# aharley/pips

Hardware: AMD Instinct MI355X
Metric: particle-updates/sec (B*S*N*iters/s) at S=8 N=256 368x496 (higher is better)
Workload: dtype f32; 1 GPU; BASELINE configs[1]: B=1/GPU S=8 368x496 N=256 I=6 fp32 stride 8, encoder included, inputs resident in HBM; clips_per_gpu=1, parallelism=clip-sharded x1, collective=none

## Files before the change

__graft_entry__.py:

```python
from __future__ import annotations

import os
import sys

ROOT = os.path.dirname(os.path.abspath(__file__))
if ROOT not in sys.path:
    sys.path.insert(0, ROOT)


def build() -> None:
    from pips_amd import _build
    lib = _build.build_library()
    assert os.path.exists(lib)
    import pips_amd
    from pips_amd import _lib
    _lib.load()
    from oracle import reference_shim
    if reference_shim.available() and os.environ.get("PIPS_SKIP_REF_CHECK") != "1":
        import subprocess
        subprocess.check_call([sys.executable, os.path.join(ROOT, "oracle", "check_against_reference.py")])


def smoke() -> None:
    import torch
    from pips_amd import Pips
    from pips_amd.weights import init_state_dict
    from oracle import pips_oracle as O

    assert torch.cuda.is_available(), "smoke() needs cuda:0"
    sd = init_state_dict(0, tamed=True)
    g = torch.Generator().manual_seed(1)
    B, N, H, W, iters = 1, 16, 128, 160, 3
    rgbs = torch.randint(0, 256, (B, 8, 3, H, W), generator=g).float()
    xys = torch.rand(B, N, 2, generator=g) * torch.tensor([W - 1.0, H - 1.0])
    m = Pips(S=8, stride=8)
    m.load_state_dict(sd)
# ... 15 lines not shown
```

pips_amd/csrc/api.hip:

```cpp
#include "common.h"

#include <cstdarg>
#include <cstdio>
#include <cstdlib>
#include <cstring>
#include <mutex>

namespace pips {

static thread_local char g_err[512] = "";

void set_error(const char* fmt, ...) {
    va_list ap;
    va_start(ap, fmt);
    vsnprintf(g_err, sizeof(g_err), fmt, ap);
    va_end(ap);
}

#ifdef PIPS_TUNING
int tune_env(const char* name, int dflt) {
    const char* e = getenv(name);
    return e ? atoi(e) : dflt;
}
#endif
// ... 367 lines not shown
}
const float* conv_w(const float* arena, const ArenaLayout& A, int ci, MatMode mode) {
    if (mode == EXACT) return arena + A.conv[ci].w;
    const unsigned short* hb = reinterpret_cast<const unsigned short*>(arena + A.total);
    return reinterpret_cast<const float*>(mode == BF16 ? hb + A.h_conv[ci] : hb + A.total_h + A.t_conv[ci]);
}

struct Enc {
    const float* arena; const ArenaLayout& A;
    int F; float* ws; const EncPlan& P; hipStream_t st; MatMode mode;
};

ConvCall enc_conv(const Enc& e, int ci, const void* in, int H, int W, void* out, bool out_bf16) {
    const ConvW& c = e.A.conv[ci];
    const MatMode lm = layer_mm(c, e.F, H, W, e.mode);
    ConvCall cc = conv_call(in, e.F, H, W, c.cin, conv_w(e.arena, e.A, ci, lm), e.arena + c.b, c.cout, c.k, c.stride, c.pad, out,
                            nullptr, nullptr);
    cc.mode = lm;
    cc.in_bf16 = e.mode == BF16;
    cc.out_bf16 = out_bf16;
    return cc;
}

int conv_stats(const Enc& e, int ci, const void* in, const float* in_norm, int H, int W, void* out, float* partial,
               float* mean_rstd) {
    const ConvW& c = e.A.conv[ci];
    int tiles = 0;
    ConvCall cc = enc_conv(e, ci, in, H, W, out, e.mode == BF16);
    cc.stats = partial; cc.tiles = &tiles; cc.in_norm = in_norm;
    if (e.mode == BF16) cc.parts_cap = enc_parts_cap(conv_out(H, c.k, c.stride, c.pad), conv_out(W, c.k, c.stride, c.pad));
    RUN(conv_nhwc(cc, e.st));
    return launch_inorm_finalize_pivot(partial, e.F, tiles, c.cout, mean_rstd, e.st);
}

int inorm_apply(const Enc& e, const void* x, const float* stats, const void* res, const float* res_stats, void* y, int HW, int C) {
    if (e.mode == BF16)
        return launch_inorm_apply_bf16(x, stats, res, res_stats, res == nullptr ? 0 : res_stats == nullptr ? 1 : 2, y, e.F, HW, C, e.st);
    return launch_inorm_apply((const float*)x, stats, (const float*)res, res_stats, (float*)y, e.F, HW, C, e.st);
}

int res_block(const Enc& e, int& ci, bool down, const void* x, int H, int W, void* out) {
    const int i1 = ci++, i2 = ci++;
    const ConvW& c1 = e.A.conv[i1];
    const ConvW& c2 = e.A.conv[i2];
    const int Ho = conv_out(H, 3, c1.stride, 1), Wo = conv_out(W, 3, c1.stride, 1);
    float* ws = e.ws; const EncPlan& P = e.P;
    void* raw = ws + P.raw; void* mid = ws + P.mid;
    RUN(conv_stats(e, i1, x, nullptr, H, W, raw, ws + P.partial, ws + P.st_a));
    RUN(inorm_apply(e, raw, ws + P.st_a, nullptr, nullptr, mid, Ho * Wo, c1.cout));
    RUN(conv_stats(e, i2, mid, nullptr, Ho, Wo, raw, ws + P.partial, ws + P.st_a));
    if (down) {
        const int id = ci++;
        RUN(conv_stats(e, id, x, nullptr, H, W, ws + P.ds, ws + P.partial2, ws + P.st_b));
        return inorm_apply(e, raw, ws + P.st_a, ws + P.ds, ws + P.st_b, out, Ho * Wo, c2.cout);
    }
    return inorm_apply(e, raw, ws + P.st_a, x, nullptr, out, Ho * Wo, c2.cout);
}

int enc_front_f32(const Enc& e, const void* rgbs, int rgb_u8, int H, int W, int& ci) {
    float* ws = e.ws; const EncPlan& P = e.P;
    const int H0 = P.Hs[0], W0 = P.Ws[0];
    int tiles = 0;
    RUN(launch_stem(rgbs, rgb_u8, e.arena + e.A.conv[0].w, e.arena + e.A.conv[0].b, ws + P.raw, ws + P.partial, e.F, H, W, H0, W0,
                    &tiles, e.st));
    RUN(launch_inorm_finalize_pivot(ws + P.partial, e.F, tiles, 64, ws + P.st_a, e.st));
    RUN(launch_inorm_apply(ws + P.raw, ws + P.st_a, nullptr, nullptr, ws + P.xa, e.F, H0 * W0, 64, e.st));
    RUN(res_block(e, ci, false, ws + P.xa, H0, W0, ws + P.xb));
    return res_block(e, ci, false, ws + P.xb, H0, W0, ws + P.outs[0]);
}

int enc_front_bf16(const Enc& e, const void* rgbs, int rgb_u8, int H, int W, int& ci) {
    float* ws = e.ws; const EncPlan& P = e.P; const ArenaLayout& A = e.A; hipStream_t st = e.st;
// ... 22 lines not shown
    RUN(check_geometry(F, H, W, stride));
    const EncPlan P = plan_encoder(F, H, W, stride);
    if (workspace_bytes < P.total * sizeof(float)) {
        set_error("encoder: workspace %zu < %zu bytes", workspace_bytes, P.total * sizeof(float));
        return PIPS_E_WORKSPACE;
    }
    float* ws = (float*)workspace;
    const Enc e = {(const float*)arena_v, arena_layout(), F, ws, P, st, encoder_mode(flags)};
    const bool h = e.mode == BF16;
    const int rgb_u8 = (flags & PIPS_FLAG_RGB_U8) ? 1 : 0;

    int ci = 1;
    RUN(h ? enc_front_bf16(e, rgbs, rgb_u8, H, W, ci) : enc_front_f32(e, rgbs, rgb_u8, H, W, ci));
    const void* x = ws + P.outs[0];
    int Hc = P.Hs[0], Wc = P.Ws[0];
    for (int l = 1; l < 4; ++l) {
        RUN(res_block(e, ci, true, x, Hc, Wc, ws + P.xb));
        Hc = P.Hs[l]; Wc = P.Ws[l];
        RUN(res_block(e, ci, false, ws + P.xb, Hc, Wc, ws + P.outs[l]));
        x = ws + P.outs[l];
    }
    const int ch[4] = {64, 96, 128, 128};
    const int H8 = P.Hs[4], W8 = P.Ws[4];
    for (int l = 0, coff = 0; l < 4; coff += ch[l], ++l)
        RUN(h ? launch_resize_into_bf16(ws + P.outs[l], F, P.Hs[l], P.Ws[l], ch[l], ws + P.cat, H8, W8, 416, coff, st)
              : launch_resize_into(ws + P.outs[l], F, P.Hs[l], P.Ws[l], ch[l], ws + P.cat, H8, W8, 416, coff, st));
    const int i2 = ci++, i3 = ci++;
    RUN(conv_stats(e, i2, ws + P.cat, nullptr, H8, W8, ws + P.raw, ws + P.partial, ws + P.st_a));
    RUN(inorm_apply(e, ws + P.raw, ws + P.st_a, nullptr, nullptr, ws + P.mid, H8 * W8, 256));
    RUN(conv_nhwc(enc_conv(e, i3, ws + P.mid, H8, W8, pyramid, false), st));
    const PyramidView v = pyramid_view(F, H8, W8);
    for (int l = 1; l < PIPS_LEVELS; ++l)
        RUN(launch_avgpool2(pyramid + v.off[l - 1], F, v.lh[l - 1], v.lw[l - 1], PIPS_C, pyramid + v.off[l], st));
    if (h) RUN(launch_pyramid_mirror(pyramid, v.levels, pyramid + v.levels, st));
    return PIPS_OK;
}

enum GatherRoute { GATHER_AUTO, GATHER_DIRECT, GATHER_TILED };

struct GatherCall {
    const float* pyramid; int B, T, R, S, H8, W8;
    const float* ffeats; const float* coords; const float* times; int N;
    const int* win_start; const int* win_dir;
    float* X;
    bool bf16_maps; GatherRoute route;
    void* scratch; size_t scratch_bytes; hipEvent_t* ev;
    hipStream_t st;
};

int mixer_input(const GatherCall& g) {
    PIPS_CHECK_ARG(g.pyramid && g.ffeats && g.coords && g.times && g.X, "mixer_input: null pointer");
    PIPS_CHECK_ARG(g.T >= 1 && g.R >= 1 && g.B > 0 && g.N > 0, "mixer_input: need T, R, B, N >= 1");
    PIPS_CHECK_ARG(g.S >= 1 && g.S <= PIPS_S_MAX, "mixer_input: window length S=%d outside 1..%d", g.S, PIPS_S_MAX);
    const PyramidView v = pyramid_view(g.B * g.R, g.H8, g.W8);
// ... 216 lines not shown
    hipStream_t st;
};

int track_impl(const TrackCall& c) {
    PIPS_CHECK_ARG(c.arena && c.pyramid && c.xys && c.times && c.workspace && c.out_trajs && c.out_vis, "track: null pointer");
    PIPS_CHECK_ARG(c.B > 0 && c.N > 0 && c.T >= 1 && c.R >= 1 && c.iters >= 0 && c.stride >= 1,
                   "track: need B,N,T,R,stride >= 1 and iters >= 0");
    PIPS_CHECK_ARG(c.S >= 1 && c.S <= PIPS_S_MAX, "track: window length S=%d outside 1..%d", c.S, PIPS_S_MAX);
    PIPS_CHECK_ARG(c.H8 >= 8 && c.W8 >= 8, "track: map %dx%d too small for a 4-level pyramid", c.H8, c.W8);
    PIPS_CHECK_ARG(c.win_dir == nullptr || c.win_start != nullptr, "track: win_dir needs win_start");
    const int B = c.B, N = c.N, S = c.S;
    const TrackPlan P = plan_track(B, N, S);
    if (c.workspace_bytes < P.total * sizeof(float)) {
        set_error("track: workspace %zu < %zu bytes", c.workspace_bytes, P.total * sizeof(float));
        return PIPS_E_WORKSPACE;
    }
    hipStream_t st = c.st;
    const float* arena = (const float*)c.arena;
    float* ws = (float*)c.workspace;
    const int M = B * N * S;
    float* coords = ws + P.coords; float* coords0 = ws + P.coords0; float* ffeats = ws + P.ffeats;
    float* ffeat0 = c.out_ffeat0 != nullptr ? c.out_ffeat0 : ws + P.ffeat0;
    const size_t traj_sz = (size_t)B * S * N * 2;
    RUN(launch_init_coords(c.xys, c.coords_init, B, N, (float)c.stride, coords, coords0, c.out_trajs, st, S));
    if (c.feat_init != nullptr) {
        if (c.feat_init != ffeat0)
            (void)hipMemcpyAsync(ffeat0, c.feat_init, (size_t)B * N * PIPS_C * sizeof(float), hipMemcpyDeviceToDevice, st);
    } else {
        RUN(launch_point_sample_strided(c.pyramid, B, c.R, c.T, c.H8, c.W8, coords, S * 2, N, c.win_start, ffeat0, st));
    }
    RUN(launch_init_ffeats(ffeat0, B * N, ffeats, st, S));
    if (c.ce_tgt != nullptr) {
        PIPS_CHECK_ARG(c.ce_terms && c.ce_ws && c.win_start == nullptr && c.T == S && c.R == c.T,
                       "track: score-map terms need their output and workspace, S frames per clip and no windows");
        if (c.ce_ws_bytes < score_map_workspace_bytes(B, c.T, c.H8, c.W8)) {
            set_error("track: score-map workspace %zu < %zu bytes", c.ce_ws_bytes, score_map_workspace_bytes(B, c.T, c.H8, c.W8));
            return PIPS_E_WORKSPACE;
        }
        RUN(score_map_prepare(c.pyramid, B, c.T, c.H8, c.W8, (float*)c.ce_ws, st));
    }
    if (c.iters == 0)
        RUN(launch_vis_head(arena, ffeats, B, N, c.out_vis, st, S));
    GatherCall g;
    memset(&g, 0, sizeof(g));
    g.pyramid = c.pyramid; g.B = B; g.T = c.T; g.R = c.R; g.S = S; g.H8 = c.H8; g.W8 = c.W8;
    g.ffeats = ffeats; g.coords = coords; g.times = c.times; g.N = N;
    g.win_start = c.win_start; g.win_dir = c.win_dir;
    g.X = ws + P.X;
    g.bf16_maps = (c.flags & PIPS_FLAG_BF16_MAPS) != 0;
    g.route = GATHER_AUTO;
    g.scratch = ws + P.mixer; g.scratch_bytes = mixer_workspace_bytes(M, S);
    g.st = st;
    for (int it = 0; it < c.iters; ++it) {
        if (c.ce_tgt != nullptr)
// ... 384 lines not shown
```

pips_amd/csrc/common.h:

```cpp
#pragma once
#include <hip/hip_runtime.h>
#include <atomic>
#include <stdint.h>
#include <stddef.h>
#include "../../include/pips_hip.h"

namespace pips {

void set_error(const char* fmt, ...);

#define PIPS_CHECK_ARG(cond, ...)                                   \
    do {                                                            \
        if (!(cond)) { ::pips::set_error(__VA_ARGS__); return PIPS_E_ARG; } \
    } while (0)

#define PIPS_CHECK_LAUNCH(what)                                                     \
    do {                                                                            \
        hipError_t e__ = hipGetLastError();                                         \
        if (e__ != hipSuccess) {                                                    \
            ::pips::set_error("%s: %s", what, hipGetErrorString(e__));              \
            return PIPS_E_LAUNCH;                                                   \
        }                                                                           \
    } while (0)

// ... 237 lines not shown
    size_t w_in, b_in;
    MixLayerW mix[PIPS_DEPTH];
    size_t lnf_g, lnf_b, w_head, b_head;
    size_t norm_g, norm_b, w_upd_t, b_upd, w_vis, b_vis;
    size_t total;
    size_t h_w1[PIPS_DEPTH], h_w2[PIPS_DEPTH], h_head, h_conv[22], h_in, total_h;
    size_t t_in, t_w1[PIPS_DEPTH], t_w2[PIPS_DEPTH], t_head, t_conv[22], total_t;
    int S, nout, nout_pad;
    size_t total_all;
};
const ArenaLayout& arena_layout(int S = PIPS_S);

inline int conv_out(int x, int k, int s, int p) { return (x + 2 * p - k) / s + 1; }

int launch_stem(const void* rgbs, int rgb_u8, const float* w, const float* bias, float* out, float* stats,
                int F, int H, int W, int Ho, int Wo, int* tiles_m, hipStream_t st);
int stem_tiles_m(int Ho, int Wo);
int launch_inorm_finalize_pivot(const float* partial, int F, int parts, int C, float* mean_rstd, hipStream_t st);
int launch_inorm_apply(const float* x, const float* stats, const float* res, const float* res_stats,
                       float* y, int F, int HW, int C, hipStream_t st);
int launch_resize_into(const float* src, int F, int Hs, int Ws, int C, float* dst, int Hd, int Wd,
                       int Cdst, int coff, hipStream_t st);
int launch_avgpool2(const float* src, int F, int H, int W, int C, float* dst, hipStream_t st);
int launch_resize_frames(const void* src, int src_u8, int planes, int h, int w, float* dst, int H, int W, hipStream_t st);
int launch_stem_bf16(const void* rgbs, int rgb_u8, const float* w, const float* bias, void* out_bf16, float* stats,
                     int F, int H, int W, int Ho, int Wo, int* tiles_m, hipStream_t st);
int launch_inorm_apply_bf16(const void* x, const float* stats, const void* res, const float* res_stats, int mode,
                            void* y, int F, int HW, int C, hipStream_t st);
int launch_resize_into_bf16(const void* src, int F, int Hs, int Ws, int C, void* dst, int Hd, int Wd, int Cdst, int coff,
                            hipStream_t st);

int launch_point_sample(const float* level0, int B, int S, int H8, int W8, const float* xy, int N,
                        float* out, hipStream_t st);
int launch_point_sample_strided(const float* level0, int B, int S, int T, int H8, int W8, const float* xy,
                                int xy_stride, int N, const int* win_start, float* out, hipStream_t st);
int launch_init_coords(const float* xys, const float* coords_init, int B, int N, float stride,
                       float* coords, float* coords0, float* out_traj0, hipStream_t st, int Sw = PIPS_S);
int launch_init_ffeats(const float* ffeat0, int BN, float* ffeats, hipStream_t st, int Sw = PIPS_S);
int launch_mixer_input(const float* pyramid, const size_t* lvl_off, const int* lvlH, const int* lvlW,
                       int B, int S, int T, const float* ffeats, const float* coords, const float* times,
                       int N, const int* win_start, const int* win_dir, float* X, hipStream_t st, int Sw = PIPS_S);
int launch_mixer_input_bf16maps(const void* mirror, const size_t* lvl_off, const int* lvlH, const int* lvlW, int B, int S,
                                int T, const float* ffeats, const float* coords, const float* times, int N,
                                const int* win_start, const int* win_dir, float* X, hipStream_t st, int Sw = PIPS_S);
int launch_pyramid_mirror(const float* pyramid, size_t floats, void* mirror, hipStream_t st);
int launch_pyramid_append(const float* src, const size_t* src_off, int k, float* dst, const size_t* dst_off, void* dst_mirror,
                          const int* pf8, int R, int T0, hipStream_t st);
size_t tiled_gather_scratch_bytes(int B, int N, int H8, int W8);
bool tiled_gather_wanted(int B, int N, int H8, int W8, bool bf16_maps = false);
int launch_mixer_input_tiled(const float* pyramid, const size_t* lvl_off, const int* lvlH, const int* lvlW, int B,
                             int S, const float* ffeats, const float* coords, const float* times, int N,
                             float* X, void* scratch, size_t scratch_bytes, hipStream_t st, hipEvent_t* ev = nullptr,
                             const unsigned short* mirror = nullptr);
int launch_token_mix(const float* arena, const MixLayerW& L, float* x, float* xn, int particles,
                     hipStream_t st, int xn_bf16 = 0, int Sw = PIPS_S, int x_bf16 = 0);
int launch_ln_mean(const float* x, const float* g, const float* b, float* out, int particles,
                   hipStream_t st, int Sw = PIPS_S, int x_bf16 = 0);
int launch_score_upsum(const float* pyramid, const size_t* lvl_off, const int* lvlH, const int* lvlW, int F, float* U,
                       hipStream_t st);
int launch_score_terms(const float* U, int B, int S, int H8, int W8, const float* ffeats, int N, const float* tgt,
                       float* out, hipStream_t st);
// ... 7 lines not shown
```

pips_amd/csrc/encoder.hip:

```cpp
#include "common.h"

namespace pips {

constexpr int STEM_ROWS = 4, STEM_COLS = 64;
constexpr int STEM_TH = 2 * STEM_ROWS + 5, STEM_TW = 136;
constexpr int STEM_STEPS = 3 * 7 * 4;
constexpr int STEM_LDS = (3 * STEM_TH * STEM_TW + STEM_STEPS * 64 * 2) * 4;

template <typename RGB, bool V4>
__global__ __launch_bounds__(256, 2) void stem_conv_kernel(const RGB* __restrict__ rgbs,
                                                           const float* __restrict__ w,
                                                           const float* __restrict__ bias,
                                                           float* __restrict__ out,
                                                           float* __restrict__ stats, int H, int W,
                                                           int Ho, int Wo, int tiles_x, int tiles, int F) {
    extern __shared__ __attribute__((aligned(16))) float stem_sm[];
    float* tile = stem_sm;
    float* wl = stem_sm + 3 * STEM_TH * STEM_TW;
    const int tid = threadIdx.x, lane = tid & 63, wave = tid >> 6;
    const int l31 = lane & 31, half = lane >> 5;
    for (int i = tid; i < STEM_STEPS * 64 * 2; i += 256) {
        const int h = i & 1, n = (i >> 1) & 63, s = i >> 7;
        const int j = s & 3, ck = s >> 2, kw = 2 * j + h - (V4 ? 1 : 0);
        wl[i] = (kw >= 0 && kw < 7) ? w[(ck * 7 + kw) * 64 + n] : 0.f;
// ... 109 lines not shown
int launch_stem(const void* rgbs, int rgb_u8, const float* w, const float* bias, float* out, float* stats,
                int F, int H, int W, int Ho, int Wo, int* tiles_m, hipStream_t st) {
    const int tiles_x = cdiv(Wo, STEM_COLS), tiles = cdiv(Ho, STEM_ROWS) * tiles_x;
    if (tiles_m) *tiles_m = stem_tiles_m(Ho, Wo);
    const int grid = tiles * F < 512 ? tiles * F : 512;
    static std::atomic<unsigned long long> raised_f{0}, raised_u{0};
    static std::atomic<unsigned long long> raised_f4{0}, raised_u4{0};
    const bool v4 = W % 4 == 0 && reinterpret_cast<uintptr_t>(rgbs) % (rgb_u8 ? 4 : 16) == 0 && PIPS_TUNE("PIPS_STEM_V4", 1);
#define PIPS_STEM32(T_, V_, RAISED_)                                                                                             \
    {                                                                                                                            \
        const int rc = ensure_dynamic_lds(RAISED_, (const void*)stem_conv_kernel<T_, V_>, STEM_LDS);                            \
        if (rc != PIPS_OK) return rc;                                                                                            \
        hipLaunchKernelGGL((stem_conv_kernel<T_, V_>), dim3(grid), dim3(256), STEM_LDS, st, (const T_*)rgbs, w, bias, out, stats, \
                           H, W, Ho, Wo, tiles_x, tiles, F);                                                                     \
    }
    if (rgb_u8) { if (v4) PIPS_STEM32(unsigned char, true, raised_u4) else PIPS_STEM32(unsigned char, false, raised_u) }
    else { if (v4) PIPS_STEM32(float, true, raised_f4) else PIPS_STEM32(float, false, raised_f) }
#undef PIPS_STEM32
    PIPS_CHECK_LAUNCH("stem_conv_kernel");
    return PIPS_OK;
}

template <int SUBS>
__global__ __launch_bounds__(4 * SUBS) void inorm_finalize_pivot_kernel(const float4* __restrict__ partial, int parts, int C,
                                                                        float* __restrict__ mean_rstd) {
    constexpr int NW = 4 * SUBS / 64;
    __shared__ double red[3][NW][4];
    const int f = blockIdx.x, cl = threadIdx.x & 3, c = blockIdx.y * 4 + cl, sub = threadIdx.x >> 2;
    const float4* p = partial + (size_t)f * parts * C + c;
    const double r = (double)p[0].z;
    double n = 0.0, s1 = 0.0, s2 = 0.0;
    for (int t0 = sub; t0 < parts; t0 += 8 * SUBS) {
        float4 v[8];
#pragma unroll
        for (int u = 0; u < 8; ++u) {
            const int t = t0 + SUBS * u;
            v[u] = t < parts ? p[(size_t)t * C] : make_float4(0.f, 0.f, 0.f, 0.f);
        }
#pragma unroll
        for (int u = 0; u < 8; ++u)
            if (v[u].w > 0.f) {
                const double nt = v[u].w, d = (double)v[u].z - r;
                n += nt;
                s1 += (double)v[u].x + nt * d;
                s2 += (double)v[u].y + d * (2.0 * (double)v[u].x + nt * d);
            }
    }
#pragma unroll
    for (int o = 4; o < 64; o <<= 1) {
        n += __shfl_xor(n, o); s1 += __shfl_xor(s1, o); s2 += __shfl_xor(s2, o);
    }
    const int wave = threadIdx.x >> 6;
    if ((threadIdx.x & 63) < 4) { red[0][wave][cl] = n; red[1][wave][cl] = s1; red[2][wave][cl] = s2; }
    __syncthreads();
    if (threadIdx.x < 4) {
        n = 0.0; s1 = 0.0; s2 = 0.0;
        for (int i = 0; i < NW; ++i) { n += red[0][i][cl]; s1 += red[1][i][cl]; s2 += red[2][i][cl]; }
        const double m1 = n > 0.0 ? s1 / n : 0.0;
        double var = n > 0.0 ? s2 / n - m1 * m1 : 0.0;
        if (var < 0.0) var = 0.0;
        mean_rstd[((size_t)f * C + c) * 2 + 0] = (float)(r + m1);
        mean_rstd[((size_t)f * C + c) * 2 + 1] = (float)(1.0 / sqrt(var + 1e-5));
    }
}

__global__ __launch_bounds__(1024) void inorm_finalize_pivot16_kernel(const float4* __restrict__ partial, int parts, int C,
                                                                    float* __restrict__ mean_rstd) {
    __shared__ double red[3][64][16];
    const int f = blockIdx.x, cl = threadIdx.x & 15, c = blockIdx.y * 16 + cl, sub = threadIdx.x >> 4;
    const float4* p = partial + (size_t)f * parts * C + c;
    const double r = (double)p[0].z;
    double n = 0.0, s1 = 0.0, s2 = 0.0;
    for (int t0 = sub; t0 < parts; t0 += 256) {
        float4 v[4];
#pragma unroll
        for (int u = 0; u < 4; ++u) {
            const int t = t0 + 64 * u;
            v[u] = t < parts ? p[(size_t)t * C] : make_float4(0.f, 0.f, 0.f, 0.f);
        }
#pragma unroll
        for (int u = 0; u < 4; ++u)
            if (v[u].w > 0.f) {
                const double nt = v[u].w, d = (double)v[u].z - r;
                n += nt;
                s1 += (double)v[u].x + nt * d;
                s2 += (double)v[u].y + d * (2.0 * (double)v[u].x + nt * d);
            }
    }
    red[0][sub][cl] = n; red[1][sub][cl] = s1; red[2][sub][cl] = s2;
    __syncthreads();
    if (sub == 0) {
        n = 0.0; s1 = 0.0; s2 = 0.0;
        for (int i = 0; i < 64; ++i) { n += red[0][i][cl]; s1 += red[1][i][cl]; s2 += red[2][i][cl]; }
        const double m1 = n > 0.0 ? s1 / n : 0.0;
        double var = n > 0.0 ? s2 / n - m1 * m1 : 0.0;
        if (var < 0.0) var = 0.0;
        mean_rstd[((size_t)f * C + c) * 2 + 0] = (float)(r + m1);
        mean_rstd[((size_t)f * C + c) * 2 + 1] = (float)(1.0 / sqrt(var + 1e-5));
    }
}

int launch_inorm_finalize_pivot(const float* partial, int F, int parts, int C, float* mean_rstd, hipStream_t st) {
    PIPS_CHECK_ARG(C % 16 == 0, "inorm_finalize: C=%d must be a multiple of 16", C);
    if (F <= 16)
        hipLaunchKernelGGL(inorm_finalize_pivot_kernel<256>, dim3(F, C / 4), dim3(1024), 0, st, reinterpret_cast<const float4*>(partial),
                           parts, C, mean_rstd);
    else
        hipLaunchKernelGGL(inorm_finalize_pivot16_kernel, dim3(F, C / 16), dim3(1024), 0, st, reinterpret_cast<const float4*>(partial),
                           parts, C, mean_rstd);
    PIPS_CHECK_LAUNCH("inorm_finalize_pivot_kernel");
    return PIPS_OK;
}

template <int MODE>
__global__ __launch_bounds__(256) void inorm_apply_kernel(const float4* __restrict__ x,
                                                          const float2* __restrict__ stats,
                                                          const float4* __restrict__ res,
                                                          const float2* __restrict__ res_stats,
                                                          float4* __restrict__ y, int HW, int C4,
                                                          size_t total4) {
    const size_t per_frame = (size_t)HW * C4;
    for (size_t i = (size_t)blockIdx.x * blockDim.x + threadIdx.x; i < total4;
         i += (size_t)gridDim.x * blockDim.x) {
        const int f = (int)(i / per_frame);
        const int c4 = (int)(i % C4);
        const float2* st = stats + ((size_t)f * C4 + c4) * 4;
        float4 v = x[i];
        float o[4] = {v.x, v.y, v.z, v.w};
#pragma unroll
        for (int k = 0; k < 4; ++k) o[k] = fmaxf((o[k] - st[k].x) * st[k].y, 0.f);
        if (MODE == 1) {
            const float4 r = res[i];
            o[0] = fmaxf(r.x + o[0], 0.f); o[1] = fmaxf(r.y + o[1], 0.f);
// ... 9 lines not shown
    }
}

int launch_inorm_apply(const float* x, const float* stats, const float* res, const float* res_stats,
                       float* y, int F, int HW, int C, hipStream_t st) {
    PIPS_CHECK_ARG(C % 4 == 0, "inorm_apply: C %% 4");
    const size_t total4 = (size_t)F * HW * (C / 4);
    const int blocks = (int)((total4 + 255) / 256 < 4096 ? (total4 + 255) / 256 : 4096);
    const float4* x4 = reinterpret_cast<const float4*>(x);
    const float2* s2 = reinterpret_cast<const float2*>(stats);
    const float4* r4 = reinterpret_cast<const float4*>(res);
    const float2* rs2 = reinterpret_cast<const float2*>(res_stats);
    float4* y4 = reinterpret_cast<float4*>(y);
    if (res == nullptr)
        hipLaunchKernelGGL(inorm_apply_kernel<0>, dim3(blocks), dim3(256), 0, st, x4, s2, r4, rs2, y4, HW, C / 4, total4);
    else if (res_stats == nullptr)
        hipLaunchKernelGGL(inorm_apply_kernel<1>, dim3(blocks), dim3(256), 0, st, x4, s2, r4, rs2, y4, HW, C / 4, total4);
    else
        hipLaunchKernelGGL(inorm_apply_kernel<2>, dim3(blocks), dim3(256), 0, st, x4, s2, r4, rs2, y4, HW, C / 4, total4);
    PIPS_CHECK_LAUNCH("inorm_apply_kernel");
    return PIPS_OK;
}

__global__ __launch_bounds__(256) void resize_into_kernel(const float* __restrict__ src, int Hs, int Ws,
                                                          int C4, float4* __restrict__ dst, int Hd,
                                                          int Wd, int Cdst4, int coff4, float sh,
                                                          float sw, size_t total4) {
    for (size_t i = (size_t)blockIdx.x * blockDim.x + threadIdx.x; i < total4;
         i += (size_t)gridDim.x * blockDim.x) {
        const int c4 = (int)(i % C4);
        size_t p = i / C4;
        const int x = (int)(p % Wd); p /= Wd;
        const int y = (int)(p % Hd);
        const int f = (int)(p / Hd);
        int y0, y1, x0, x1;
        float ly0, ly1, lx0, lx1;
        if (Hd == Hs) { y0 = y1 = y; ly0 = 1.f; ly1 = 0.f; }
        else {
            const float r = sh * (float)y;
            y0 = min((int)floorf(r), Hs - 1);
            ly1 = fminf(fmaxf(r - (float)y0, 0.f), 1.f);
            y1 = y0 + (y0 < Hs - 1 ? 1 : 0);
            ly0 = 1.f - ly1;
        }
        if (Wd == Ws) { x0 = x1 = x; lx0 = 1.f; lx1 = 0.f; }
        else {
            const float r = sw * (float)x;
            x0 = min((int)floorf(r), Ws - 1);
            lx1 = fminf(fmaxf(r - (float)x0, 0.f), 1.f);
            x1 = x0 + (x0 < Ws - 1 ? 1 : 0);
            lx0 = 1.f - lx1;
        }
        const float4* s4 = reinterpret_cast<const float4*>(src) + (size_t)f * Hs * Ws * C4 + c4;
        const float4 v00 = s4[((size_t)y0 * Ws + x0) * C4], v01 = s4[((size_t)y0 * Ws + x1) * C4];
        const float4 v10 = s4[((size_t)y1 * Ws + x0) * C4], v11 = s4[((size_t)y1 * Ws + x1) * C4];
        float4 o;
        o.x = ly0 * (lx0 * v00.x + lx1 * v01.x) + ly1 * (lx0 * v10.x + lx1 * v11.x);
        o.y = ly0 * (lx0 * v00.y + lx1 * v01.y) + ly1 * (lx0 * v10.y + lx1 * v11.y);
        o.z = ly0 * (lx0 * v00.z + lx1 * v01.z) + ly1 * (lx0 * v10.z + lx1 * v11.z);
        o.w = ly0 * (lx0 * v00.w + lx1 * v01.w) + ly1 * (lx0 * v10.w + lx1 * v11.w);
        dst[(((size_t)f * Hd + y) * Wd + x) * Cdst4 + coff4 + c4] = o;
    }
}

int launch_resize_into(const float* src, int F, int Hs, int Ws, int C, float* dst, int Hd, int Wd,
                       int Cdst, int coff, hipStream_t st) {
    PIPS_CHECK_ARG(C % 4 == 0 && Cdst % 4 == 0 && coff % 4 == 0, "resize: channel alignment");
    const size_t total4 = (size_t)F * Hd * Wd * (C / 4);
    const int blocks = (int)((total4 + 255) / 256 < 4096 ? (total4 + 255) / 256 : 4096);
    const float sh = Hd > 1 ? (float)(Hs - 1) / (float)(Hd - 1) : 0.f;
    const float sw = Wd > 1 ? (float)(Ws - 1) / (float)(Wd - 1) : 0.f;
    hipLaunchKernelGGL(resize_into_kernel, dim3(blocks), dim3(256), 0, st, src, Hs, Ws, C / 4,
                       reinterpret_cast<float4*>(dst), Hd, Wd, Cdst / 4, coff / 4, sh, sw, total4);
    PIPS_CHECK_LAUNCH("resize_into_kernel");
    return PIPS_OK;
}

__global__ __launch_bounds__(256) void avgpool2_kernel(const float4* __restrict__ src, int H, int W,
                                                       int C4, float4* __restrict__ dst, int Ho, int Wo,
                                                       size_t total4) {
    for (size_t i = (size_t)blockIdx.x * blockDim.x + threadIdx.x; i < total4;
         i += (size_t)gridDim.x * blockDim.x) {
        const int c4 = (int)(i % C4);
        size_t p = i / C4;
        const int x = (int)(p % Wo); p /= Wo;
        const int y = (int)(p % Ho);
        const int f = (int)(p / Ho);
        const float4* s = src + (((size_t)f * H + 2 * y) * W + 2 * x) * C4 + c4;
        const float4 a = s[0], b = s[C4], c = s[(size_t)W * C4], d = s[(size_t)W * C4 + C4];
        float4 o;
        o.x = (((a.x + b.x) + c.x) + d.x) * 0.25f;
        o.y = (((a.y + b.y) + c.y) + d.y) * 0.25f;
        o.z = (((a.z + b.z) + c.z) + d.z) * 0.25f;
        o.w = (((a.w + b.w) + c.w) + d.w) * 0.25f;
        dst[i] = o;
    }
}

int launch_avgpool2(const float* src, int F, int H, int W, int C, float* dst, hipStream_t st) {
    const int Ho = H / 2, Wo = W / 2;
    PIPS_CHECK_ARG(Ho >= 1 && Wo >= 1, "avgpool: map %dx%d too small", H, W);
    const size_t total4 = (size_t)F * Ho * Wo * (C / 4);
    const int blocks = (int)((total4 + 255) / 256 < 4096 ? (total4 + 255) / 256 : 4096);
    hipLaunchKernelGGL(avgpool2_kernel, dim3(blocks), dim3(256), 0, st,
                       reinterpret_cast<const float4*>(src), H, W, C / 4,
                       reinterpret_cast<float4*>(dst), Ho, Wo, total4);
    PIPS_CHECK_LAUNCH("avgpool2_kernel");
    return PIPS_OK;
}

template <typename T>
__global__ __launch_bounds__(256) void resize_frames_kernel(const T* __restrict__ src, int planes, int h, int w,
                                                            float* __restrict__ dst, int H, int W, float sh, float sw) {
    const size_t i = (size_t)blockIdx.x * blockDim.x + threadIdx.x;
    if (i >= (size_t)planes * H * W) return;
    const int x = (int)(i % W), y = (int)((i / W) % H);
    const size_t pl = i / ((size_t)W * H);
    const float fy = fmaxf(__fsub_rn(__fmul_rn(sh, (float)y + 0.5f), 0.5f), 0.f);
    const float fx = fmaxf(__fsub_rn(__fmul_rn(sw, (float)x + 0.5f), 0.5f), 0.f);
    const int y0 = (int)fy, x0 = (int)fx;
    const int y1 = y0 + (y0 < h - 1 ? 1 : 0), x1 = x0 + (x0 < w - 1 ? 1 : 0);
    const float ly1 = fy - (float)y0, lx1 = fx - (float)x0, ly0 = 1.f - ly1, lx0 = 1.f - lx1;
    const T* p = src + pl * (size_t)h * w;
    const float p00 = (float)p[(size_t)y0 * w + x0], p01 = (float)p[(size_t)y0 * w + x1];
    const float p10 = (float)p[(size_t)y1 * w + x0], p11 = (float)p[(size_t)y1 * w + x1];
    const float top = __fadd_rn(__fmul_rn(lx0, p00), __fmul_rn(lx1, p01));
    const float bot = __fadd_rn(__fmul_rn(lx0, p10), __fmul_rn(lx1, p11));
    dst[i] = __fadd_rn(__fmul_rn(ly0, top), __fmul_rn(ly1, bot));
}

int launch_resize_frames(const void* src, int src_u8, int planes, int h, int w, float* dst, int H, int W, hipStream_t st) {
    const size_t total = (size_t)planes * H * W;
    const float sh = (float)h / (float)H, sw = (float)w / (float)W;
// ... 13 lines not shown
```

pips_amd/csrc/track.hip:

```cpp
#include "common.h"

namespace pips {

constexpr int S = PIPS_S;
constexpr int C = PIPS_C;


__global__ __launch_bounds__(128) void point_sample_kernel(const float* __restrict__ level0, int S_, int T_,
                                                           int H, int W, const float* __restrict__ xy,
                                                           int xy_stride, int N,
                                                           const int* __restrict__ win_start,
                                                           float* __restrict__ out) {
    const int pn = blockIdx.x;
    const int b = pn / N;
    const float x = xy[(size_t)pn * xy_stride + 0], y = xy[(size_t)pn * xy_stride + 1];
    const float x0f = floorf(x), y0f = floorf(y);
    const float x1f = x0f + 1.f, y1f = y0f + 1.f;
    const int x0 = min(max((int)x0f, 0), W - 1), x1 = min(max((int)x0f + 1, 0), W - 1);
    const int y0 = min(max((int)y0f, 0), H - 1), y1 = min(max((int)y0f + 1, 0), H - 1);
    const float w00 = __fmul_rn(x1f - x, y1f - y), w01 = __fmul_rn(x - x0f, y1f - y);
    const float w10 = __fmul_rn(x1f - x, y - y0f), w11 = __fmul_rn(x - x0f, y - y0f);
    const int f_first = win_start != nullptr ? ring_slot(min(max(win_start[pn], 0), T_ - 1), S_) : 0;
    const float* f0 = level0 + ((size_t)b * S_ + f_first) * H * W * C;
    const int c = threadIdx.x;
// ... 41 lines not shown
    const size_t i = (size_t)blockIdx.x * blockDim.x + threadIdx.x;
    if (i >= (size_t)BN * Sw * (C / 4)) return;
    const size_t pn = i / ((size_t)Sw * (C / 4));
    ffeats[i] = ffeat0[pn * (C / 4) + (i % (C / 4))];
}

int launch_init_coords(const float* xys, const float* coords_init, int B, int N, float stride,
                       float* coords, float* coords0, float* out_traj0, hipStream_t st, int Sw) {
    const int total = B * N * Sw;
    hipLaunchKernelGGL(init_coords_kernel, dim3(cdiv(total, 256)), dim3(256), 0, st, xys, coords_init, B,
                       N, Sw, stride, coords, coords0, out_traj0);
    PIPS_CHECK_LAUNCH("init_coords_kernel");
    return PIPS_OK;
}

int launch_init_ffeats(const float* ffeat0, int BN, float* ffeats, hipStream_t st, int Sw) {
    const size_t total = (size_t)BN * Sw * (C / 4);
    hipLaunchKernelGGL(init_ffeats_kernel, dim3((unsigned)((total + 255) / 256)), dim3(256), 0, st,
                       reinterpret_cast<const float4*>(ffeat0), BN, Sw, reinterpret_cast<float4*>(ffeats));
    PIPS_CHECK_LAUNCH("init_ffeats_kernel");
    return PIPS_OK;
}

struct LevelTable {
    size_t off[PIPS_LEVELS];
    int H[PIPS_LEVELS], W[PIPS_LEVELS];
};

template <int SCT>
__global__ __launch_bounds__(256) __attribute__((amdgpu_waves_per_eu(2, 4))) void mixer_input_kernel(const float* __restrict__ pyramid,
                                                          LevelTable lv, int S_, int T_, int Srt,
                                                          const float* __restrict__ ffeats,
                                                          const float* __restrict__ coords,
                                                          const float* __restrict__ times, int N,
                                                          const int* __restrict__ win_start,
                                                          const int* __restrict__ win_dir,
                                                          float* __restrict__ X) {
    __shared__ float Dw[PIPS_LEVELS][64];
    const int S = SCT ? SCT : Srt;
    const int m = blockIdx.x;
    const int s = m % S, pn = m / S;
    const int b = pn / N;
    int fstart = 0, dir = 1;
    if (win_start != nullptr) {
        fstart = win_start[pn];
        if (win_dir != nullptr) dir = win_dir[pn] < 0 ? -1 : 1;
// ... 1088 lines not shown
```

Baseline: 1.381 million particle-updates/s.

## Fuse small encoder and tracker-prologue kernels to cut launch count

Several small launches are merged. The two instance-norm finalizes in downsampling residual blocks share one kernel. The four feature-map resizes into the concat buffer become one kernel. The three pyramid avgpool levels are built in one pass through shared memory. Coordinate init, point sampling and ffeat broadcast run as a single prologue kernel. The aim is to remove launch overhead and intermediate re-reads, at the cost of more complex kernels with a different per-thread layout, all gated behind a tuning flag that defaults to on.

```diff
diff --git a/__graft_entry__.py b/__graft_entry__.py
--- a/__graft_entry__.py
+++ b/__graft_entry__.py
@@ -12,6 +12,7 @@
     from pips_amd import _build
     lib = _build.build_library()
     assert os.path.exists(lib)
+    assert os.path.exists(_build.build_library(tuning=True))
     import pips_amd
     from pips_amd import _lib
     _lib.load()
diff --git a/pips_amd/csrc/api.hip b/pips_amd/csrc/api.hip
--- a/pips_amd/csrc/api.hip
+++ b/pips_amd/csrc/api.hip
@@ -413,15 +413,20 @@
     return cc;
 }
 
+bool enc_fuse() { return PIPS_TUNE("PIPS_ENC_FUSE", 1) != 0; }
+
+int conv_partials(const Enc& e, int ci, const void* in, const float* in_norm, int H, int W, void* out, float* partial, int* tiles) {
+    const ConvW& c = e.A.conv[ci];
+    ConvCall cc = enc_conv(e, ci, in, H, W, out, e.mode == BF16);
+    cc.stats = partial; cc.tiles = tiles; cc.in_norm = in_norm;
+    if (e.mode == BF16) cc.parts_cap = enc_parts_cap(conv_out(H, c.k, c.stride, c.pad), conv_out(W, c.k, c.stride, c.pad));
+    return conv_nhwc(cc, e.st);
+}
 int conv_stats(const Enc& e, int ci, const void* in, const float* in_norm, int H, int W, void* out, float* partial,
                float* mean_rstd) {
-    const ConvW& c = e.A.conv[ci];
     int tiles = 0;
-    ConvCall cc = enc_conv(e, ci, in, H, W, out, e.mode == BF16);
-    cc.stats = partial; cc.tiles = &tiles; cc.in_norm = in_norm;
-    if (e.mode == BF16) cc.parts_cap = enc_parts_cap(conv_out(H, c.k, c.stride, c.pad), conv_out(W, c.k, c.stride, c.pad));
-    RUN(conv_nhwc(cc, e.st));
-    return launch_inorm_finalize_pivot(partial, e.F, tiles, c.cout, mean_rstd, e.st);
+    RUN(conv_partials(e, ci, in, in_norm, H, W, out, partial, &tiles));
+    return launch_inorm_finalize_pivot(partial, e.F, tiles, e.A.conv[ci].cout, mean_rstd, e.st);
 }
 
 int inorm_apply(const Enc& e, const void* x, const float* stats, const void* res, const float* res_stats, void* y, int HW, int C) {
@@ -439,6 +444,15 @@
     void* raw = ws + P.raw; void* mid = ws + P.mid;
     RUN(conv_stats(e, i1, x, nullptr, H, W, raw, ws + P.partial, ws + P.st_a));
     RUN(inorm_apply(e, raw, ws + P.st_a, nullptr, nullptr, mid, Ho * Wo, c1.cout));
+    if (down && enc_fuse()) {
+        const int id = ci++;
+        int t2 = 0, td = 0;
+        RUN(conv_partials(e, i2, mid, nullptr, Ho, Wo, raw, ws + P.partial, &t2));
+        RUN(conv_partials(e, id, x, nullptr, H, W, ws + P.ds, ws + P.partial2, &td));
+        RUN(launch_inorm_finalize_pivot2(ws + P.partial, t2, c2.cout, ws + P.st_a, ws + P.partial2, td, e.A.conv[id].cout,
+                                         ws + P.st_b, e.F, e.st));
+        return inorm_apply(e, raw, ws + P.st_a, ws + P.ds, ws + P.st_b, out, Ho * Wo, c2.cout);
+    }
     RUN(conv_stats(e, i2, mid, nullptr, Ho, Wo, raw, ws + P.partial, ws + P.st_a));
     if (down) {
         const int id = ci++;
@@ -507,6 +521,10 @@
     }
     const int ch[4] = {64, 96, 128, 128};
     const int H8 = P.Hs[4], W8 = P.Ws[4];
+    if (!h && enc_fuse()) {
+        const float* srcs[4] = {ws + P.outs[0], ws + P.outs[1], ws + P.outs[2], ws + P.outs[3]};
+        RUN(launch_resize_into4(srcs, P.Hs, P.Ws, ch, F, ws + P.cat, H8, W8, 416, st));
+    } else
     for (int l = 0, coff = 0; l < 4; coff += ch[l], ++l)
         RUN(h ? launch_resize_into_bf16(ws + P.outs[l], F, P.Hs[l], P.Ws[l], ch[l], ws + P.cat, H8, W8, 416, coff, st)
               : launch_resize_into(ws + P.outs[l], F, P.Hs[l], P.Ws[l], ch[l], ws + P.cat, H8, W8, 416, coff, st));
@@ -515,6 +533,10 @@
     RUN(inorm_apply(e, ws + P.raw, ws + P.st_a, nullptr, nullptr, ws + P.mid, H8 * W8, 256));
     RUN(conv_nhwc(enc_conv(e, i3, ws + P.mid, H8, W8, pyramid, false), st));
     const PyramidView v = pyramid_view(F, H8, W8);
+    static_assert(PIPS_LEVELS == 4, "launch_avgpool2_x3 writes levels 1..3");
+    if (enc_fuse())
+        RUN(launch_avgpool2_x3(pyramid + v.off[0], F, v.lh[0], v.lw[0], pyramid + v.off[1], pyramid + v.off[2], pyramid + v.off[3], st));
+    else
     for (int l = 1; l < PIPS_LEVELS; ++l)
         RUN(launch_avgpool2(pyramid + v.off[l - 1], F, v.lh[l - 1], v.lw[l - 1], PIPS_C, pyramid + v.off[l], st));
     if (h) RUN(launch_pyramid_mirror(pyramid, v.levels, pyramid + v.levels, st));
@@ -777,14 +799,19 @@
     float* coords = ws + P.coords; float* coords0 = ws + P.coords0; float* ffeats = ws + P.ffeats;
     float* ffeat0 = c.out_ffeat0 != nullptr ? c.out_ffeat0 : ws + P.ffeat0;
     const size_t traj_sz = (size_t)B * S * N * 2;
-    RUN(launch_init_coords(c.xys, c.coords_init, B, N, (float)c.stride, coords, coords0, c.out_trajs, st, S));
-    if (c.feat_init != nullptr) {
-        if (c.feat_init != ffeat0)
-            (void)hipMemcpyAsync(ffeat0, c.feat_init, (size_t)B * N * PIPS_C * sizeof(float), hipMemcpyDeviceToDevice, st);
+    if (enc_fuse()) {
+        RUN(launch_track_prologue(c.xys, c.coords_init, c.feat_init, c.pyramid, B, c.R, c.T, c.H8, c.W8, N, (float)c.stride,
+                                  c.win_start, coords, coords0, c.out_trajs, ffeat0, ffeats, st, S));
     } else {
-        RUN(launch_point_sample_strided(c.pyramid, B, c.R, c.T, c.H8, c.W8, coords, S * 2, N, c.win_start, ffeat0, st));
-    }
-    RUN(launch_init_ffeats(ffeat0, B * N, ffeats, st, S));
+        RUN(launch_init_coords(c.xys, c.coords_init, B, N, (float)c.stride, coords, coords0, c.out_trajs, st, S));
+        if (c.feat_init != nullptr) {
+            if (c.feat_init != ffeat0)
+                (void)hipMemcpyAsync(ffeat0, c.feat_init, (size_t)B * N * PIPS_C * sizeof(float), hipMemcpyDeviceToDevice, st);
+        } else {
+            RUN(launch_point_sample_strided(c.pyramid, B, c.R, c.T, c.H8, c.W8, coords, S * 2, N, c.win_start, ffeat0, st));
+        }
+        RUN(launch_init_ffeats(ffeat0, B * N, ffeats, st, S));
+    }
     if (c.ce_tgt != nullptr) {
         PIPS_CHECK_ARG(c.ce_terms && c.ce_ws && c.win_start == nullptr && c.T == S && c.R == c.T,
                        "track: score-map terms need their output and workspace, S frames per clip and no windows");
diff --git a/pips_amd/csrc/common.h b/pips_amd/csrc/common.h
--- a/pips_amd/csrc/common.h
+++ b/pips_amd/csrc/common.h
@@ -283,6 +283,11 @@
 int launch_resize_into(const float* src, int F, int Hs, int Ws, int C, float* dst, int Hd, int Wd,
                        int Cdst, int coff, hipStream_t st);
 int launch_avgpool2(const float* src, int F, int H, int W, int C, float* dst, hipStream_t st);
+int launch_inorm_finalize_pivot2(const float* partial_a, int parts_a, int Ca, float* mean_rstd_a, const float* partial_b,
+                                 int parts_b, int Cb, float* mean_rstd_b, int F, hipStream_t st);
+int launch_resize_into4(const float* const* srcs, const int* Hs, const int* Ws, const int* C, int F, float* dst, int Hd, int Wd,
+                        int Cdst, hipStream_t st);
+int launch_avgpool2_x3(const float* l0, int F, int H0, int W0, float* l1, float* l2, float* l3, hipStream_t st);
 int launch_resize_frames(const void* src, int src_u8, int planes, int h, int w, float* dst, int H, int W, hipStream_t st);
 int launch_stem_bf16(const void* rgbs, int rgb_u8, const float* w, const float* bias, void* out_bf16, float* stats,
                      int F, int H, int W, int Ho, int Wo, int* tiles_m, hipStream_t st);
@@ -298,6 +303,9 @@
 int launch_init_coords(const float* xys, const float* coords_init, int B, int N, float stride,
                        float* coords, float* coords0, float* out_traj0, hipStream_t st, int Sw = PIPS_S);
 int launch_init_ffeats(const float* ffeat0, int BN, float* ffeats, hipStream_t st, int Sw = PIPS_S);
+int launch_track_prologue(const float* xys, const float* coords_init, const float* feat_init, const float* level0, int B, int R_,
+                          int T_, int H8, int W8, int N, float stride, const int* win_start, float* coords, float* coords0,
+                          float* out_traj0, float* ffeat0, float* ffeats, hipStream_t st, int Sw = PIPS_S);
 int launch_mixer_input(const float* pyramid, const size_t* lvl_off, const int* lvlH, const int* lvlW,
                        int B, int S, int T, const float* ffeats, const float* coords, const float* times,
                        int N, const int* win_start, const int* win_dir, float* X, hipStream_t st, int Sw = PIPS_S);
diff --git a/pips_amd/csrc/encoder.hip b/pips_amd/csrc/encoder.hip
--- a/pips_amd/csrc/encoder.hip
+++ b/pips_amd/csrc/encoder.hip
@@ -155,11 +155,11 @@
 }
 
 template <int SUBS>
-__global__ __launch_bounds__(4 * SUBS) void inorm_finalize_pivot_kernel(const float4* __restrict__ partial, int parts, int C,
-                                                                        float* __restrict__ mean_rstd) {
+__device__ __forceinline__ void inorm_finalize_pivot_block(const float4* __restrict__ partial, int parts, int C,
+                                                           float* __restrict__ mean_rstd, int f, int cg) {
     constexpr int NW = 4 * SUBS / 64;
     __shared__ double red[3][NW][4];
-    const int f = blockIdx.x, cl = threadIdx.x & 3, c = blockIdx.y * 4 + cl, sub = threadIdx.x >> 2;
+    const int cl = threadIdx.x & 3, c = cg * 4 + cl, sub = threadIdx.x >> 2;
     const float4* p = partial + (size_t)f * parts * C + c;
     const double r = (double)p[0].z;
     double n = 0.0, s1 = 0.0, s2 = 0.0;
@@ -197,6 +197,21 @@
     }
 }
 
+template <int SUBS>
+__global__ __launch_bounds__(4 * SUBS) void inorm_finalize_pivot_kernel(const float4* __restrict__ partial, int parts, int C,
+                                                                        float* __restrict__ mean_rstd) {
+    inorm_finalize_pivot_block<SUBS>(partial, parts, C, mean_rstd, blockIdx.x, blockIdx.y);
+}
+
+struct InormSet { const float4* partial; int parts, C; float* mean_rstd; };
+template <int SUBS>
+__global__ __launch_bounds__(4 * SUBS) void inorm_finalize_pivot2_kernel(InormSet a, InormSet b) {
+    const int ga = a.C / 4, y = blockIdx.y;
+    const bool second = y >= ga;
+    inorm_finalize_pivot_block<SUBS>(second ? b.partial : a.partial, second ? b.parts : a.parts, second ? b.C : a.C,
+                                     second ? b.mean_rstd : a.mean_rstd, blockIdx.x, second ? y - ga : y);
+}
+
 __global__ __launch_bounds__(1024) void inorm_finalize_pivot16_kernel(const float4* __restrict__ partial, int parts, int C,
                                                                     float* __restrict__ mean_rstd) {
     __shared__ double red[3][64][16];
@@ -242,6 +257,20 @@
         hipLaunchKernelGGL(inorm_finalize_pivot16_kernel, dim3(F, C / 16), dim3(1024), 0, st, reinterpret_cast<const float4*>(partial),
                            parts, C, mean_rstd);
     PIPS_CHECK_LAUNCH("inorm_finalize_pivot_kernel");
+    return PIPS_OK;
+}
+
+int launch_inorm_finalize_pivot2(const float* partial_a, int parts_a, int Ca, float* mean_rstd_a, const float* partial_b,
+                                 int parts_b, int Cb, float* mean_rstd_b, int F, hipStream_t st) {
+    if (F > 16) {
+        const int rc = launch_inorm_finalize_pivot(partial_a, F, parts_a, Ca, mean_rstd_a, st);
+        return rc != PIPS_OK ? rc : launch_inorm_finalize_pivot(partial_b, F, parts_b, Cb, mean_rstd_b, st);
+    }
+    PIPS_CHECK_ARG(Ca % 16 == 0 && Cb % 16 == 0, "inorm_finalize: C=%d / %d must be multiples of 16", Ca, Cb);
+    const InormSet a = {reinterpret_cast<const float4*>(partial_a), parts_a, Ca, mean_rstd_a};
+    const InormSet b = {reinterpret_cast<const float4*>(partial_b), parts_b, Cb, mean_rstd_b};
+    hipLaunchKernelGGL(inorm_finalize_pivot2_kernel<256>, dim3(F, Ca / 4 + Cb / 4), dim3(1024), 0, st, a, b);
+    PIPS_CHECK_LAUNCH("inorm_finalize_pivot2_kernel");
     return PIPS_OK;
 }
 
@@ -297,6 +326,37 @@
     return PIPS_OK;
 }
 
+__device__ __forceinline__ float4 resize_pixel(const float* __restrict__ src, int Hs, int Ws, int C4, int Hd, int Wd, float sh,
+                                               float sw, int f, int y, int x, int c4) {
+    int y0, y1, x0, x1;
+    float ly0, ly1, lx0, lx1;
+    if (Hd == Hs) { y0 = y1 = y; ly0 = 1.f; ly1 = 0.f; }
+    else {
+        const float r = sh * (float)y;
+        y0 = min((int)floorf(r), Hs - 1);
+        ly1 = fminf(fmaxf(r - (float)y0, 0.f), 1.f);
+        y1 = y0 + (y0 < Hs - 1 ? 1 : 0);
+        ly0 = 1.f - ly1;
+    }
+    if (Wd == Ws) { x0 = x1 = x; lx0 = 1.f; lx1 = 0.f; }
+    else {
+        const float r = sw * (float)x;
+        x0 = min((int)floorf(r), Ws - 1);
+        lx1 = fminf(fmaxf(r - (float)x0, 0.f), 1.f);
+        x1 = x0 + (x0 < Ws - 1 ? 1 : 0);
+        lx0 = 1.f - lx1;
+    }
+    const float4* s4 = reinterpret_cast<const float4*>(src) + (size_t)f * Hs * Ws * C4 + c4;
+    const float4 v00 = s4[((size_t)y0 * Ws + x0) * C4], v01 = s4[((size_t)y0 * Ws + x1) * C4];
+    const float4 v10 = s4[((size_t)y1 * Ws + x0) * C4], v11 = s4[((size_t)y1 * Ws + x1) * C4];
+    float4 o;
+    o.x = ly0 * (lx0 * v00.x + lx1 * v01.x) + ly1 * (lx0 * v10.x + lx1 * v11.x);
+    o.y = ly0 * (lx0 * v00.y + lx1 * v01.y) + ly1 * (lx0 * v10.y + lx1 * v11.y);
+    o.z = ly0 * (lx0 * v00.z + lx1 * v01.z) + ly1 * (lx0 * v10.z + lx1 * v11.z);
+    o.w = ly0 * (lx0 * v00.w + lx1 * v01.w) + ly1 * (lx0 * v10.w + lx1 * v11.w);
+    return o;
+}
+
 __global__ __launch_bounds__(256) void resize_into_kernel(const float* __restrict__ src, int Hs, int Ws,
                                                           int C4, float4* __restrict__ dst, int Hd,
                                                           int Wd, int Cdst4, int coff4, float sh,
@@ -308,33 +368,28 @@
         const int x = (int)(p % Wd); p /= Wd;
         const int y = (int)(p % Hd);
         const int f = (int)(p / Hd);
-        int y0, y1, x0, x1;
-        float ly0, ly1, lx0, lx1;
-        if (Hd == Hs) { y0 = y1 = y; ly0 = 1.f; ly1 = 0.f; }
-        else {
-            const float r = sh * (float)y;
-            y0 = min((int)floorf(r), Hs - 1);
-            ly1 = fminf(fmaxf(r - (float)y0, 0.f), 1.f);
-            y1 = y0 + (y0 < Hs - 1 ? 1 : 0);
-            ly0 = 1.f - ly1;
-        }
-        if (Wd == Ws) { x0 = x1 = x; lx0 = 1.f; lx1 = 0.f; }
-        else {
-            const float r = sw * (float)x;
-            x0 = min((int)floorf(r), Ws - 1);
-            lx1 = fminf(fmaxf(r - (float)x0, 0.f), 1.f);
-            x1 = x0 + (x0 < Ws - 1 ? 1 : 0);
-            lx0 = 1.f - lx1;
-        }
-        const float4* s4 = reinterpret_cast<const float4*>(src) + (size_t)f * Hs * Ws * C4 + c4;
-        const float4 v00 = s4[((size_t)y0 * Ws + x0) * C4], v01 = s4[((size_t)y0 * Ws + x1) * C4];
-        const float4 v10 = s4[((size_t)y1 * Ws + x0) * C4], v11 = s4[((size_t)y1 * Ws + x1) * C4];
-        float4 o;
-        o.x = ly0 * (lx0 * v00.x + lx1 * v01.x) + ly1 * (lx0 * v10.x + lx1 * v11.x);
-        o.y = ly0 * (lx0 * v00.y + lx1 * v01.y) + ly1 * (lx0 * v10.y + lx1 * v11.y);
-        o.z = ly0 * (lx0 * v00.z + lx1 * v01.z) + ly1 * (lx0 * v10.z + lx1 * v11.z);
-        o.w = ly0 * (lx0 * v00.w + lx1 * v01.w) + ly1 * (lx0 * v10.w + lx1 * v11.w);
-        dst[(((size_t)f * Hd + y) * Wd + x) * Cdst4 + coff4 + c4] = o;
+        dst[(((size_t)f * Hd + y) * Wd + x) * Cdst4 + coff4 + c4] = resize_pixel(src, Hs, Ws, C4, Hd, Wd, sh, sw, f, y, x, c4);
+    }
+}
+
+struct ResizeSrc { const float* src; int Hs, Ws, C4, coff4; float sh, sw; };
+struct ResizeSrc4 { ResizeSrc s[4]; };
+__global__ __launch_bounds__(256) void resize_into4_kernel(ResizeSrc4 t, float4* __restrict__ dst, int Hd, int Wd, int Cdst4,
+                                                           size_t total4) {
+    for (size_t i = (size_t)blockIdx.x * blockDim.x + threadIdx.x; i < total4;
+         i += (size_t)gridDim.x * blockDim.x) {
+        const int cc = (int)(i % Cdst4);
+        size_t p = i / Cdst4;
+        const int x = (int)(p % Wd); p /= Wd;
+        const int y = (int)(p % Hd);
+        const int f = (int)(p / Hd);
+        const int l = (cc >= t.s[1].coff4) + (cc >= t.s[2].coff4) + (cc >= t.s[3].coff4);
+#define PIPS_SEL(m) (l == 0 ? t.s[0].m : l == 1 ? t.s[1].m : l == 2 ? t.s[2].m : t.s[3].m)
+        const float* src = PIPS_SEL(src);
+        const int Hs = PIPS_SEL(Hs), Ws = PIPS_SEL(Ws), C4 = PIPS_SEL(C4), coff4 = PIPS_SEL(coff4);
+        const float sh = PIPS_SEL(sh), sw = PIPS_SEL(sw);
+#undef PIPS_SEL
+        dst[i] = resize_pixel(src, Hs, Ws, C4, Hd, Wd, sh, sw, f, y, x, cc - coff4);
     }
 }
 
@@ -348,6 +403,25 @@
     hipLaunchKernelGGL(resize_into_kernel, dim3(blocks), dim3(256), 0, st, src, Hs, Ws, C / 4,
                        reinterpret_cast<float4*>(dst), Hd, Wd, Cdst / 4, coff / 4, sh, sw, total4);
     PIPS_CHECK_LAUNCH("resize_into_kernel");
+    return PIPS_OK;
+}
+
+int launch_resize_into4(const float* const* srcs, const int* Hs, const int* Ws, const int* C, int F, float* dst, int Hd, int Wd,
+                        int Cdst, hipStream_t st) {
+    ResizeSrc4 t;
+    int coff = 0;
+    for (int l = 0; l < 4; ++l) {
+        PIPS_CHECK_ARG(C[l] > 0 && C[l] % 4 == 0, "resize: channel alignment");
+        t.s[l] = {srcs[l], Hs[l], Ws[l], C[l] / 4, coff / 4, Hd > 1 ? (float)(Hs[l] - 1) / (float)(Hd - 1) : 0.f,
+                  Wd > 1 ? (float)(Ws[l] - 1) / (float)(Wd - 1) : 0.f};
+        coff += C[l];
+    }
+    PIPS_CHECK_ARG(coff == Cdst, "resize: the sources hold %d channels, the destination %d", coff, Cdst);
+    const size_t total4 = (size_t)F * Hd * Wd * (Cdst / 4);
+    const int blocks = (int)((total4 + 255) / 256 < 16384 ? (total4 + 255) / 256 : 16384);
+    hipLaunchKernelGGL(resize_into4_kernel, dim3(blocks), dim3(256), 0, st, t, reinterpret_cast<float4*>(dst), Hd, Wd, Cdst / 4,
+                       total4);
+    PIPS_CHECK_LAUNCH("resize_into4_kernel");
     return PIPS_OK;
 }
 
@@ -384,6 +458,60 @@
     return PIPS_OK;
 }
 
+__global__ __launch_bounds__(256) void avgpool2_x3_kernel(const float4* __restrict__ l0, int H0, int W0, float4* __restrict__ l1,
+                                                          float4* __restrict__ l2, float4* __restrict__ l3) {
+    constexpr int C4 = PIPS_C / 4;
+    __shared__ float4 p1[16][C4], p2[4][C4];
+    const int H1 = H0 / 2, W1 = W0 / 2, H2 = H1 / 2, W2 = W1 / 2, H3 = H2 / 2, W3 = W2 / 2;
+    const int f = blockIdx.z, by = blockIdx.y, bx = blockIdx.x;
+    const int c4 = threadIdx.x & (C4 - 1), g = threadIdx.x >> 5;
+    auto avg4 = [](const float4 a, const float4 b, const float4 c, const float4 d) {
+        float4 o;
+        o.x = (((a.x + b.x) + c.x) + d.x) * 0.25f;
+        o.y = (((a.y + b.y) + c.y) + d.y) * 0.25f;
+        o.z = (((a.z + b.z) + c.z) + d.z) * 0.25f;
+        o.w = (((a.w + b.w) + c.w) + d.w) * 0.25f;
+        return o;
+    };
+    float4 v[2][4];
+    bool ok[2];
+#pragma unroll
+    for (int u = 0; u < 2; ++u) {
+        const int p = g + 8 * u, y = 4 * by + (p >> 2), x = 4 * bx + (p & 3);
+        ok[u] = y < H1 && x < W1;
+        const float4* s = l0 + (((size_t)f * H0 + (ok[u] ? 2 * y : 0)) * W0 + (ok[u] ? 2 * x : 0)) * C4 + c4;
+        v[u][0] = s[0]; v[u][1] = s[C4]; v[u][2] = s[(size_t)W0 * C4]; v[u][3] = s[(size_t)W0 * C4 + C4];
+    }
+#pragma unroll
+    for (int u = 0; u < 2; ++u) {
+        const int p = g + 8 * u, y = 4 * by + (p >> 2), x = 4 * bx + (p & 3);
+        const float4 o = ok[u] ? avg4(v[u][0], v[u][1], v[u][2], v[u][3]) : make_float4(0.f, 0.f, 0.f, 0.f);
+        p1[p][c4] = o;
+        if (ok[u]) l1[(((size_t)f * H1 + y) * W1 + x) * C4 + c4] = o;
+    }
+    __syncthreads();
+    if (g < 4) {
+        const int qy = g >> 1, qx = g & 1, y = 2 * by + qy, x = 2 * bx + qx;
+        const int p = (2 * qy) * 4 + 2 * qx;
+        const float4 o = avg4(p1[p][c4], p1[p + 1][c4], p1[p + 4][c4], p1[p + 5][c4]);
+        p2[g][c4] = o;
+        if (y < H2 && x < W2) l2[(((size_t)f * H2 + y) * W2 + x) * C4 + c4] = o;
+    }
+    __syncthreads();
+    if (g == 0 && by < H3 && bx < W3)
+        l3[(((size_t)f * H3 + by) * W3 + bx) * C4 + c4] = avg4(p2[0][c4], p2[1][c4], p2[2][c4], p2[3][c4]);
+}
+
+int launch_avgpool2_x3(const float* l0, int F, int H0, int W0, float* l1, float* l2, float* l3, hipStream_t st) {
+    const int H1 = H0 / 2, W1 = W0 / 2;
+    PIPS_CHECK_ARG(H1 / 4 >= 1 && W1 / 4 >= 1, "avgpool: map %dx%d too small for three more levels", H0, W0);
+    PIPS_CHECK_ARG(F <= 65535 && cdiv(H1, 4) <= 65535, "avgpool: grid too large");
+    hipLaunchKernelGGL(avgpool2_x3_kernel, dim3(cdiv(W1, 4), cdiv(H1, 4), F), dim3(256), 0, st, reinterpret_cast<const float4*>(l0),
+                       H0, W0, reinterpret_cast<float4*>(l1), reinterpret_cast<float4*>(l2), reinterpret_cast<float4*>(l3));
+    PIPS_CHECK_LAUNCH("avgpool2_x3_kernel");
+    return PIPS_OK;
+}
+
 template <typename T>
 __global__ __launch_bounds__(256) void resize_frames_kernel(const T* __restrict__ src, int planes, int h, int w,
                                                             float* __restrict__ dst, int H, int W, float sh, float sw) {
diff --git a/pips_amd/csrc/track.hip b/pips_amd/csrc/track.hip
--- a/pips_amd/csrc/track.hip
+++ b/pips_amd/csrc/track.hip
@@ -87,6 +87,62 @@
     return PIPS_OK;
 }
 
+__global__ __launch_bounds__(128) void track_prologue_kernel(const float* __restrict__ xys, const float* __restrict__ coords_init,
+                                                             const float* __restrict__ feat_init, const float* __restrict__ level0,
+                                                             int R_, int T_, int H, int W, int B, int N, int Sw, float stride,
+                                                             const int* __restrict__ win_start, float* __restrict__ coords,
+                                                             float* __restrict__ coords0, float* __restrict__ out_traj0,
+                                                             float* __restrict__ ffeat0, float* __restrict__ ffeats) {
+    const int pn = blockIdx.x, n = pn % N, b = pn / N;
+    for (int s = threadIdx.x; s < Sw; s += 128) {
+        const size_t i = (size_t)pn * Sw + s;
+        float x, y;
+        if (coords_init != nullptr) {
+            const float* p = coords_init + (((size_t)b * Sw + s) * N + n) * 2;
+            x = p[0] / stride; y = p[1] / stride;
+        } else {
+            x = xys[(size_t)pn * 2 + 0] / stride; y = xys[(size_t)pn * 2 + 1] / stride;
+        }
+        coords[i * 2 + 0] = x; coords[i * 2 + 1] = y;
+        coords0[i * 2 + 0] = x; coords0[i * 2 + 1] = y;
+        float* o = out_traj0 + (((size_t)b * Sw + s) * N + n) * 2;
+        o[0] = x * stride; o[1] = y * stride;
+    }
+    const int c = threadIdx.x;
+    float o;
+    if (feat_init != nullptr) {
+        o = feat_init[(size_t)pn * C + c];
+        if (feat_init != ffeat0) ffeat0[(size_t)pn * C + c] = o;
+    } else {
+        const float* p0 = coords_init != nullptr ? coords_init + ((size_t)b * Sw * N + n) * 2 : xys + (size_t)pn * 2;
+        const float x = p0[0] / stride, y = p0[1] / stride;
+        const float x0f = floorf(x), y0f = floorf(y);
+        const float x1f = x0f + 1.f, y1f = y0f + 1.f;
+        const int x0 = min(max((int)x0f, 0), W - 1), x1 = min(max((int)x0f + 1, 0), W - 1);
+        const int y0 = min(max((int)y0f, 0), H - 1), y1 = min(max((int)y0f + 1, 0), H - 1);
+        const float w00 = __fmul_rn(x1f - x, y1f - y), w01 = __fmul_rn(x - x0f, y1f - y);
+        const float w10 = __fmul_rn(x1f - x, y - y0f), w11 = __fmul_rn(x - x0f, y - y0f);
+        const int f_first = win_start != nullptr ? ring_slot(min(max(win_start[pn], 0), T_ - 1), R_) : 0;
+        const float* f0 = level0 + ((size_t)b * R_ + f_first) * H * W * C;
+        const float v00 = f0[((size_t)y0 * W + x0) * C + c], v01 = f0[((size_t)y0 * W + x1) * C + c];
+        const float v10 = f0[((size_t)y1 * W + x0) * C + c], v11 = f0[((size_t)y1 * W + x1) * C + c];
+        o = __fadd_rn(__fmul_rn(w00, v00), __fmul_rn(w01, v01));
+        o = __fadd_rn(o, __fmul_rn(w10, v10));
+        o = __fadd_rn(o, __fmul_rn(w11, v11));
+        ffeat0[(size_t)pn * C + c] = o;
+    }
+    for (int s = 0; s < Sw; ++s) ffeats[((size_t)pn * Sw + s) * C + c] = o;
+}
+
+int launch_track_prologue(const float* xys, const float* coords_init, const float* feat_init, const float* level0, int B, int R_,
+                          int T_, int H8, int W8, int N, float stride, const int* win_start, float* coords, float* coords0,
+                          float* out_traj0, float* ffeat0, float* ffeats, hipStream_t st, int Sw) {
+    hipLaunchKernelGGL(track_prologue_kernel, dim3(B * N), dim3(128), 0, st, xys, coords_init, feat_init, level0, R_, T_, H8, W8,
+                       B, N, Sw, stride, win_start, coords, coords0, out_traj0, ffeat0, ffeats);
+    PIPS_CHECK_LAUNCH("track_prologue_kernel");
+    return PIPS_OK;
+}
+
 struct LevelTable {
     size_t off[PIPS_LEVELS];
     int H[PIPS_LEVELS], W[PIPS_LEVELS];
```

Result: no change. 1.384 million particle-updates/s (median of 6 runs) (+0.2%).
